# vita-epfl/motion-style-transfer

Measured on AMD Instinct MI355X. Metric: trajectories/sec fwd+bwd (Y-Net+LoRA, SDD shortterm), higher is better.
Workload: dtype f32; 1 GPU; C2: SDD shortterm Y-Net + LoRA rank=1 on encoder[0-4], 256x256 raster, obs=8 pred=12; batch_per_gpu=32, global_batch=32, raster=256x256, obs_len=8, pred_len=12, train_net=mosa_1, parallelism=dp1, trainable_floats=8190

## Files before the change

motion-style-transfer_amd/csrc/lora_wgrad.hip:

```cpp
#include "ynet_common.h"
#include <stdlib.h>
#include <stdio.h>
#include <type_traits>

#define LW_RQ 3
#define LW_ROWS 9

struct LoraWgArgs {
    YSrc src[YNET_MAX_SRC];
    int nsrc, cin;
    const float* dy;
    long long dy_bs;
    const float* mask;
    long long mask_bs;
    const float* lora_a;
    const float* lora_b;
    float* partial;
    int B, H, W, cout;
    int tiles_x, tiles_y, ntiles;
#ifdef YNET_LW_PROFILE
    unsigned long long* prof;
#endif
};

#ifdef YNET_LW_PROFILE
#define LW_STAMP(i) do { __builtin_amdgcn_sched_barrier(0); unsigned long long t_; asm volatile("s_waitcnt vmcnt(0) lgkmcnt(0)\n\ts_memtime %0\n\ts_waitcnt lgkmcnt(0)" : "=s"(t_) :: "memory"); pr[i] += t_ - tp; tp = t_; __builtin_amdgcn_sched_barrier(0); } while (0)
#else
#define LW_STAMP(i) do { } while (0)
#endif

typedef __attribute__((address_space(3))) void* lw_lds_ptr_t;
typedef const __attribute__((address_space(4))) float* lw_const_f32;

template <int TH>
struct LwCfg {
    static constexpr int TW = 32, NPIX = TH * TW, NH = 256 / NPIX;
    static constexpr int TROWS = TH + 2, TCOLS = 40;
    static constexpr int XDATA = TROWS * TCOLS / 4;
    static constexpr int XQ = (XDATA + 1 + 6) / 8 * 8 + 1;
    static constexpr int XCH = XQ * 4;
    static constexpr int DCH = NPIX + 4;
    static constexpr int PL = NPIX + 4;
    static_assert(XCH % 32 == 4 && DCH % 32 == 4, "bank-spread strides");
    static_assert(NH == 2 || NH == 4, "256 threads = NH slices of the tile's pixels");
    static constexpr int KSTEPS = NPIX / 4;
};

static inline int lw_xq(int th) { return ((th + 2) * 10 + 1 + 6) / 8 * 8 + 1; }
static inline int lw_lds_floats(int th, int cin, int cout) {
    const int npix = th * 32;
    return cin * lw_xq(th) * 4 + 64 + cout * (npix + 4) + 2 * LW_ROWS * (npix + 4) + cout * 12 + cin * 28;
}

__device__ __forceinline__ void lw_dma16(__amdgpu_buffer_rsrc_t r, const float* lds, unsigned voff) {
    __builtin_amdgcn_raw_ptr_buffer_load_lds(r, (lw_lds_ptr_t)lds, 16, voff, 0, 0, 0);
}

template <int TH, int NTG, int COS, int CIN_T, int COUT_T>
__global__ __launch_bounds__(256, (TH == 2 && COS <= 8) ? 3 : 2) void lora_wgrad_kernel(const LoraWgArgs a) {
    using C = LwCfg<TH>;
    constexpr int NPIX = C::NPIX, NH = C::NH, TCOLS = C::TCOLS, XQ = C::XQ, XCH = C::XCH, DCH = C::DCH, PL = C::PL;
    extern __shared__ __attribute__((aligned(16))) float smem[];
    const int cin = CIN_T ? CIN_T : a.cin, cout = COUT_T ? COUT_T : a.cout;
    float* xs = smem;
    float* ds = xs + cin * XCH + 64;
    float* dpl = ds + cout * DCH;
    float* xpl = dpl + LW_ROWS * PL;
    float* tb = xpl + LW_ROWS * PL;
    float* ta = tb + cout * 12;

    const int tid = threadIdx.x, lane = tid & 63;
    const int wave = __builtin_amdgcn_readfirstlane(tid >> 6);
    const int H = a.H, W = a.W, HW = H * W;
    const unsigned plane_bytes = (unsigned)HW * 4u;
    const int ncol = 9 * cin;
    const int n3 = 3 * cin;
    const lw_const_f32 la = (lw_const_f32)a.lora_a;

    const int NE = (cout + 15) >> 4;
    const int r16 = lane & 15, kq = lane >> 4;
    int gbase[NTG];
#pragma unroll
    for (int j = 0; j < NTG; ++j) {
        int u = (wave + 4 * j) * 16 + r16;
        u = u < ncol ? u : ncol - 1;
        const int ci = u / 9, t = u - 9 * ci, ky = t / 3, kx = t - 3 * ky;
        gbase[j] = ci * XCH + ky * TCOLS + kx + 3 + kq;
    }
    int eco = wave * 16 + r16;
    eco = eco < cout ? eco : cout - 1;
    const int ebase = eco * DCH + kq;
    const int arow = (r16 < LW_ROWS ? r16 : LW_ROWS - 1) * PL + kq;
    const bool has_e = wave < NE;

    f32x4 accg[NTG], acce = {0.f, 0.f, 0.f, 0.f};
#pragma unroll
    for (int j = 0; j < NTG; ++j) accg[j] = f32x4{0.f, 0.f, 0.f, 0.f};

    const int p = tid & (NPIX - 1);
    const int h = __builtin_amdgcn_readfirstlane(tid / NPIX);
    const int prow = p >> 5, pcol = p & 31;
    const int xoff_p = prow * TCOLS + pcol + 3;

    constexpr int XI_MAX = TH == 4 ? 9 : 11;
    const int nquads = cin * XQ;
    int xrc[XI_MAX];
    unsigned xcoff[XI_MAX];
    int xsid[XI_MAX];
#pragma unroll
    for (int k = 0; k < XI_MAX; ++k) {
        const int q = tid + k * 256;
        const int ch = q / XQ, within = q - ch * XQ;
        const int row = within / (TCOLS / 4), colp = (within - row * (TCOLS / 4)) * 4;
        int c = ch, sid = -1;
        if (q < nquads && within < C::XDATA) {
#pragma unroll
            for (int s_ = 0; s_ < YNET_MAX_SRC; ++s_) {
                if (sid < 0 && s_ < a.nsrc) {
                    if (c < a.src[s_].c) sid = s_;
                    else c -= a.src[s_].c;
                }
            }
        }
        xrc[k] = sid >= 0 ? (row << 8 | colp) : -1;
        xcoff[k] = (unsigned)c * plane_bytes;
        xsid[k] = sid;
    }

    for (int i = tid; i < cout * 12; i += 256) {
        const int co = i / 12, m = i - 12 * co;
        tb[i] = m < LW_ROWS ? a.lora_b[9 * co + m] : 0.f;
    }
    for (int i = tid; i < cin * 28; i += 256) {
        const int ci = i / 28, j = i - 28 * ci, q = j / 9, tp = j - 9 * q;
        const int ii = (9 * ci) / n3;
        const int n = 9 * ci + tp - ii * n3;
        ta[i] = (j < 27 && n < n3) ? a.lora_a[q * n3 + n] : 0.f;
    }

    float dyv[COS], mkv[COS];
    auto fetch_dy = [&](int tile) {
        int t = tile;
        const int x0 = (t % a.tiles_x) * 32;
        t /= a.tiles_x;
        const int y0 = (t % a.tiles_y) * TH;
        const int b = t / a.tiles_y;
        const int gy = y0 + prow, gx = x0 + pcol;
        const bool inside = gy < H && gx < W;
        const long long pix = (long long)gy * W + gx;
        const float* dyp = a.dy + (long long)b * a.dy_bs + pix;
        const float* mkp = a.mask ? a.mask + (long long)b * a.mask_bs + pix : nullptr;
#pragma unroll
        for (int k = 0; k < COS; ++k) {
            const int co = h + k * NH;
            const bool ok = inside && co < cout;
            dyv[k] = ok ? dyp[(long long)co * HW] : 0.f;
            mkv[k] = (ok && mkp) ? mkp[(long long)co * HW] : 1.f;
        }
    };
    if ((int)blockIdx.x < a.ntiles) fetch_dy(blockIdx.x);
#ifdef YNET_LW_PROFILE
    unsigned long long pr[8] = {0, 0, 0, 0, 0, 0, 0, 0}, tp = __builtin_amdgcn_s_memtime();
    const unsigned long long t_begin = tp;
#endif

    for (int tile = blockIdx.x; tile < a.ntiles; tile += gridDim.x) {
        int t = tile;
        const int x0 = (t % a.tiles_x) * 32;
        t /= a.tiles_x;
        const int y0 = (t % a.tiles_y) * TH;
        const int b = t / a.tiles_y;

        {
            unsigned xo[XI_MAX];
#pragma unroll
            for (int k = 0; k < XI_MAX; ++k) {
                const int gy = y0 + (xrc[k] >> 8) - 1, gx = x0 + (xrc[k] & 255) - 4;
                const bool ok = xrc[k] >= 0 && gy >= 0 && gy < H && gx >= 0 && gx < W;
                xo[k] = ok ? xcoff[k] + (unsigned)(gy * W + gx) * 4u : 0x80000000u;
            }
#pragma unroll 1
            for (int s_ = 0; s_ < a.nsrc; ++s_) {
                const float* base = a.src[s_].p + (long long)b * a.src[s_].bs;
                const unsigned long long ub = (unsigned long long)base;
                const unsigned lo = __builtin_amdgcn_readfirstlane((unsigned)ub), hi = __builtin_amdgcn_readfirstlane((unsigned)(ub >> 32));
                const __amdgpu_buffer_rsrc_t r = __builtin_amdgcn_make_buffer_rsrc(
                    (void*)(((unsigned long long)hi << 32) | lo), 0, (unsigned)a.src[s_].c * plane_bytes, 0x00020000);
#pragma unroll
                for (int k = 0; k < XI_MAX; ++k) {
                    if (k * 256 < nquads) {
                        const int with_src = xo[k] == 0x80000000u ? 0 : xsid[k];
                        if (tid + k * 256 < nquads && with_src == s_) lw_dma16(r, xs + (k * 256 + wave * 64) * 4, xo[k]);
                    }
                }
            }
        }
        LW_STAMP(0);
        float dp[LW_ROWS], xp[LW_ROWS];
#pragma unroll
        for (int m = 0; m < LW_ROWS; ++m) dp[m] = xp[m] = 0.f;
#pragma unroll
        for (int k = 0; k < COS; ++k) {
            const int co = h + k * NH;
            if (co < cout) {
                const float d = mkv[k] > 0.f ? dyv[k] : 0.f;
                ds[co * DCH + p] = d;
                const f32x4* cb = reinterpret_cast<const f32x4*>(tb + co * 12);
                const f32x4 c0 = cb[0], c1 = cb[1], c2 = cb[2];
#pragma unroll
                for (int m = 0; m < LW_ROWS; ++m)
                    dp[m] = __builtin_fmaf(m < 4 ? c0[m & 3] : (m < 8 ? c1[m & 3] : c2[m & 3]), d, dp[m]);
            }
        }
        LW_STAMP(1);
        asm volatile("s_waitcnt vmcnt(0)" ::: "memory");
        __syncthreads();
        LW_STAMP(2);

        {
            const float* xb = xs + xoff_p;
#pragma unroll
            for (int ii = 0; ii < 3; ++ii) {
                float s0 = 0.f, s1 = 0.f, s2 = 0.f;
                const int lo_u = ii * n3, hi_u = lo_u + n3;
                const int ci_lo = (lo_u + 8) / 9, ci_hi = hi_u / 9;
                const int head_end = min(9 * ci_lo, hi_u);
                const int tail_begin = max(9 * ci_hi, head_end);
#pragma unroll 2
                for (int ci = ci_lo + h; ci < ci_hi; ci += NH) {
                    const float* xc = xb + ci * XCH;
                    const f32x4* cv = reinterpret_cast<const f32x4*>(ta + ci * 28);
                    float cf[28], xv[9];
#pragma unroll
                    for (int j = 0; j < 7; ++j) {
                        const f32x4 c4 = cv[j];
                        cf[4 * j] = c4[0];
                        cf[4 * j + 1] = c4[1];
                        cf[4 * j + 2] = c4[2];
                        cf[4 * j + 3] = c4[3];
                    }
#pragma unroll
                    for (int t = 0; t < 9; ++t) xv[t] = xc[(t / 3) * TCOLS + (t % 3)];
#pragma unroll
                    for (int t = 0; t < 9; ++t) {
                        s0 = __builtin_fmaf(cf[t], xv[t], s0);
                        s1 = __builtin_fmaf(cf[9 + t], xv[t], s1);
                        s2 = __builtin_fmaf(cf[18 + t], xv[t], s2);
                    }
                }
                if (h == 0) {
                    auto one = [&](int u) {
                        const int ci = u / 9, tp = u - 9 * ci, ky = tp / 3, kx = tp - 3 * ky, n = u - lo_u;
                        const float xv = xb[ci * XCH + ky * TCOLS + kx];
                        s0 = __builtin_fmaf(la[n], xv, s0);
                        s1 = __builtin_fmaf(la[n3 + n], xv, s1);
                        s2 = __builtin_fmaf(la[2 * n3 + n], xv, s2);
                    };
#pragma unroll 1
                    for (int u = lo_u; u < head_end; ++u) one(u);
#pragma unroll 1
                    for (int u = tail_begin; u < hi_u; ++u) one(u);
                }
                xp[3 * ii + 0] = s0;
                xp[3 * ii + 1] = s1;
                xp[3 * ii + 2] = s2;
            }
        }
        LW_STAMP(3);
#pragma unroll
        for (int hh = 0; hh < NH; ++hh) {
            if (h == hh) {
#pragma unroll
                for (int m = 0; m < LW_ROWS; ++m) {
                    if (hh == 0) {
                        dpl[m * PL + p] = dp[m];
                        xpl[m * PL + p] = xp[m];
                    } else {
                        dpl[m * PL + p] += dp[m];
                        xpl[m * PL + p] += xp[m];
                    }
                }
            }
            __syncthreads();
        }

        LW_STAMP(4);
        if (tile + (int)gridDim.x < a.ntiles) fetch_dy(tile + gridDim.x);

        LW_STAMP(5);
        {
            const float* a_dp = dpl + arow;
            const float* a_xp = xpl + arow;
            const float* b_e = ds + ebase;
            const float* b_g[NTG];
#pragma unroll
            for (int j = 0; j < NTG; ++j) b_g[j] = xs + gbase[j];
            auto run = [&](auto with_e) {
                constexpr bool WE = decltype(with_e)::value;
                float ac, bc[NTG], ec = 0.f, dc = 0.f, an, bn[NTG], en = 0.f, dn = 0.f;
                ac = a_dp[0];
#pragma unroll
                for (int j = 0; j < NTG; ++j) bc[j] = b_g[j][0];
                if (WE) {
                    ec = a_xp[0];
                    dc = b_e[0];
                }
#pragma unroll
                for (int s_ = 0; s_ < C::KSTEPS; ++s_) {
                    if (s_ + 1 < C::KSTEPS) {
                        const int sn = s_ + 1, xo = (sn >> 3) * TCOLS + (sn & 7) * 4;
                        an = a_dp[4 * sn];
#pragma unroll
                        for (int j = 0; j < NTG; ++j) bn[j] = b_g[j][xo];
                        if (WE) {
                            en = a_xp[4 * sn];
                            dn = b_e[4 * sn];
                        }
                    }
                    __builtin_amdgcn_sched_barrier(0);
#pragma unroll
                    for (int j = 0; j < NTG; ++j) accg[j] = __builtin_amdgcn_mfma_f32_16x16x4f32(ac, bc[j], accg[j], 0, 0, 0);
                    if (WE) acce = __builtin_amdgcn_mfma_f32_16x16x4f32(ec, dc, acce, 0, 0, 0);
                    __builtin_amdgcn_sched_barrier(0);
                    ac = an;
#pragma unroll
                    for (int j = 0; j < NTG; ++j) bc[j] = bn[j];
                    if (WE) {
                        ec = en;
                        dc = dn;
                    }
                }
            };
            if (has_e) run(std::true_type{});
            else run(std::false_type{});
        }
        LW_STAMP(6);
        __syncthreads();
        LW_STAMP(7);
    }
#ifdef YNET_LW_PROFILE
    if (lane == 0) {
        for (int i = 0; i < 8; ++i) atomicAdd(a.prof + i, pr[i]);
        atomicAdd(a.prof + 8, __builtin_amdgcn_s_memtime() - t_begin);
        atomicAdd(a.prof + 9, 1ull);
    }
#endif

    float* pg = a.partial + (long long)blockIdx.x * (LW_ROWS * (ncol + cout));
    float* pe = pg + LW_ROWS * ncol;
#pragma unroll
    for (int j = 0; j < NTG; ++j) {
        const int u = (wave + 4 * j) * 16 + r16;
        if (u < ncol) {
#pragma unroll
            for (int e = 0; e < 4; ++e) {
                const int m = 4 * kq + e;
                if (m < LW_ROWS) pg[m * ncol + u] = accg[j][e];
            }
        }
    }
    if (has_e) {
        const int co = wave * 16 + r16;
        if (co < cout) {
#pragma unroll
            for (int e = 0; e < 4; ++e) {
                const int m = 4 * kq + e;
                if (m < LW_ROWS) pe[m * cout + co] = acce[e];
            }
        }
    }
}

__global__ __launch_bounds__(256) void lora_wgrad_reduce_kernel(const float* __restrict__ partial, int nwg, int cin, int cout,
                                                                float scale, float* __restrict__ d_a, float* __restrict__ d_b) {
    __shared__ float red[8][32];
    const int o = threadIdx.x & 31, g = threadIdx.x >> 5;
    const int n3 = 3 * cin, ncol = 9 * cin, na = LW_RQ * n3, nb = 9 * cout;
    const long long stride = (long long)LW_ROWS * (ncol + cout);
    for (int base = blockIdx.x * 32; base < na + nb; base += gridDim.x * 32) {
        const int i = base + o;
        float s0 = 0.f, s1 = 0.f, s2 = 0.f;
        if (i < na) {
            const int q = i / n3, n = i - q * n3;
            const float* p0 = partial + (0 * LW_RQ + q) * ncol + 0 * n3 + n;
            const float* p1 = partial + (1 * LW_RQ + q) * ncol + 1 * n3 + n;
            const float* p2 = partial + (2 * LW_RQ + q) * ncol + 2 * n3 + n;
            int w = g;
            for (; w + 24 < nwg; w += 32) {
                float t0 = 0.f, t1 = 0.f, t2 = 0.f;
#pragma unroll
                for (int k = 0; k < 4; ++k) {
                    t0 += p0[(w + 8 * k) * stride];
                    t1 += p1[(w + 8 * k) * stride];
                    t2 += p2[(w + 8 * k) * stride];
                }
                s0 += t0;
                s1 += t1;
                s2 += t2;
            }
            for (; w < nwg; w += 8) {
                s0 += p0[w * stride];
                s1 += p1[w * stride];
                s2 += p2[w * stride];
            }
        } else if (i < na + nb) {
            const int f = i - na, co = f / 9, m = f - 9 * co;
            const float* p0 = partial + (long long)LW_ROWS * ncol + m * cout + co;
            int w = g;
            for (; w + 56 < nwg; w += 64) {
                float t0 = 0.f, t1 = 0.f;
#pragma unroll
                for (int k = 0; k < 4; ++k) {
                    t0 += p0[(w + 8 * k) * stride];
                    t1 += p0[(w + 32 + 8 * k) * stride];
                }
                s0 += t0;
                s1 += t1;
            }
            for (; w < nwg; w += 8) s0 += p0[w * stride];
        }
        red[g][o] = (s0 + s1) + s2;
        __syncthreads();
        if (g == 0 && i < na + nb) {
            float t = red[0][o];
#pragma unroll
            for (int k = 1; k < 8; ++k) t += red[k][o];
            if (i < na) d_a[i] = scale * t;
            else d_b[i - na] = scale * t;
        }
        __syncthreads();
    }
}

static int lw_tile_rows(int cin, int cout) {
    if (cin <= 32 && cout <= 32) return 4;
    if (cin <= 64 && cout <= 64) return 2;
    return 0;
}

static int lw_grid(int ntiles, int lds_bytes) {
    int dev = 0, cus = 256;
    (void)hipGetDevice(&dev);
    (void)hipDeviceGetAttribute(&cus, hipDeviceAttributeMultiprocessorCount, dev);
    if (cus < 1) cus = 256;
    int per_cu = (160 * 1024) / lds_bytes;
    static const int cap = getenv("YNET_LW_WG_PER_CU") ? atoi(getenv("YNET_LW_WG_PER_CU")) : 3;
    if (per_cu > cap) per_cu = cap;
    if (per_cu < 1) per_cu = 1;
    const int slots = per_cu * cus;
    return ntiles < slots ? ntiles : slots;
}

template <int TH, int NTG, int COS, int CIN_T = 0, int COUT_T = 0>
static int launch_lora_wgrad(const LoraWgArgs& a, int grid, hipStream_t st) {
    static bool attr_dev[YNET_MAX_DEV] = {false};
    bool& attr_set = attr_dev[ynet_device_slot()];
    if (!attr_set) {
        (void)hipFuncSetAttribute(reinterpret_cast<const void*>(lora_wgrad_kernel<TH, NTG, COS, CIN_T, COUT_T>), hipFuncAttributeMaxDynamicSharedMemorySize, 160 * 1024);
        attr_set = true;
    }
    const int lds = lw_lds_floats(TH, a.cin, a.cout) * 4;
#ifdef YNET_LW_PROFILE
    static unsigned long long* prof_dev = nullptr;
    if (!prof_dev) (void)hipMalloc(&prof_dev, 128);
    (void)hipMemsetAsync(prof_dev, 0, 128, st);
    LoraWgArgs ap = a;
    ap.prof = prof_dev;
    hipLaunchKernelGGL((lora_wgrad_kernel<TH, NTG, COS, CIN_T, COUT_T>), dim3(grid), dim3(256), lds, st, ap);
    {
        unsigned long long h[16];
        (void)hipMemcpyAsync(h, prof_dev, 128, hipMemcpyDeviceToHost, st);
        (void)hipStreamSynchronize(st);
        const double tot = (double)h[8];
        static const char* nm[8] = {"dma-issue", "DP", "dma-wait+barrier", "XP", "combine", "dy-prefetch", "MFMA", "end-barrier"};
        fprintf(stderr, "lora_wgrad<%d,%d,%d,%d,%d> grid %d tiles %d waves %llu avg cycles/wave %.0f:", TH, NTG, COS, CIN_T, COUT_T, grid, a.ntiles, h[9], tot / (double)h[9]);
        for (int i = 0; i < 8; ++i) fprintf(stderr, " %s %.1f%%", nm[i], 100.0 * (double)h[i] / tot);
        fprintf(stderr, "\n");
    }
#else
    hipLaunchKernelGGL((lora_wgrad_kernel<TH, NTG, COS, CIN_T, COUT_T>), dim3(grid), dim3(256), lds, st, a);
#endif
    return ynet_check_launch("lora_conv2d_wgrad");
}

extern "C" {

int ynet_lora_conv2d_wgrad_supported(int cin, int cout, int K, int r, int W) {
    static const int on = getenv("YNET_LORA_WGRAD") ? atoi(getenv("YNET_LORA_WGRAD")) : 1;
    return (on && K == 3 && r == 1 && cin >= 1 && cout >= 1 && (W & 3) == 0 && lw_tile_rows(cin, cout) != 0) ? 1 : 0;
}

int ynet_lora_conv2d_wgrad_preferred(int cin, int cout, int K, int r, int W) {
    static const int on = getenv("YNET_LORA_WGRAD") ? atoi(getenv("YNET_LORA_WGRAD")) : 1;
    if (!ynet_lora_conv2d_wgrad_supported(cin, cout, K, r, W)) return 0;
    return (on >= 2 || cout > 32) ? 1 : 0;
}

long long ynet_lora_conv2d_wgrad_workspace_floats(int cin, int cout) {
    return 1024ll * LW_ROWS * (9ll * cin + cout);
}

int ynet_lora_conv2d_wgrad(const float* const* src, const int* src_c, const long long* src_bs, int nsrc,
                           const float* dy, long long dy_bs, const float* mask, long long mask_bs,
                           const float* lora_a, const float* lora_b, float scale, float* d_a, float* d_b,
                           float* workspace, int B, int H, int W, int cout, int K, int r, void* stream) {
    YNET_REQUIRE(nsrc >= 1 && nsrc <= YNET_MAX_SRC, "lora_conv2d_wgrad: 1..%d sources supported", YNET_MAX_SRC);
    YNET_REQUIRE(dy && lora_a && lora_b && d_a && d_b && workspace, "lora_conv2d_wgrad: null pointer");
    YNET_REQUIRE(B > 0 && H > 0 && W > 0 && cout > 0, "lora_conv2d_wgrad: empty problem");
    LoraWgArgs a{};
    a.nsrc = nsrc;
    a.cin = 0;
    auto misaligned = [](const void* p, long long bs) { return (reinterpret_cast<uintptr_t>(p) & 15) != 0 || (bs & 3) != 0; };
    for (int i = 0; i < nsrc; ++i) {
        YNET_REQUIRE(src[i] != nullptr && src_c[i] > 0, "lora_conv2d_wgrad: source %d is null/empty", i);
        YNET_REQUIRE(!misaligned(src[i], src_bs[i]), "lora_conv2d_wgrad: source %d is not 16-byte aligned", i);
        a.src[i] = YSrc{src[i], src_c[i], src_bs[i], 0};
        a.cin += src_c[i];
    }
    YNET_REQUIRE(ynet_lora_conv2d_wgrad_supported(a.cin, cout, K, r, W), "lora_conv2d_wgrad: cin %d cout %d K %d r %d W %d is not served (3x3, r = 1, channels <= 64, W %% 4 == 0)", a.cin, cout, K, r, W);
    static const int th2_all = getenv("YNET_LW_TH2") ? atoi(getenv("YNET_LW_TH2")) : 0;
    const int th = th2_all ? 2 : lw_tile_rows(a.cin, cout);
    a.dy = dy;
    a.dy_bs = dy_bs;
    a.mask = mask;
    a.mask_bs = mask_bs;
    a.lora_a = lora_a;
    a.lora_b = lora_b;
    a.partial = workspace;
    a.B = B;
    a.H = H;
    a.W = W;
    a.cout = cout;
    a.tiles_x = ceil_div(W, 32);
    a.tiles_y = ceil_div(H, th);
    a.ntiles = B * a.tiles_x * a.tiles_y;
    YNET_REQUIRE(a.cin * lw_xq(th) <= (th == 4 ? 9 : 11) * 256, "lora_conv2d_wgrad: x tile of %d channels exceeds the DMA plan", a.cin);
    const int grid = lw_grid(a.ntiles, lw_lds_floats(th, a.cin, cout) * 4);
    hipStream_t st = (hipStream_t)stream;
    const int ntg = ceil_div(ceil_div(9 * a.cin, 16), 4);
    int rc;
    if (th == 2 && a.cin == 14 && cout == 32) rc = launch_lora_wgrad<2, 2, 8, 14, 32>(a, grid, st);
    else if (th == 2 && a.cin == 32 && cout == 32) rc = launch_lora_wgrad<2, 5, 8, 32, 32>(a, grid, st);
    else if (th == 2 && a.cin == 32 && cout == 64) rc = launch_lora_wgrad<2, 5, 16, 32, 64>(a, grid, st);
    else if (a.cin == 14 && cout == 32) rc = launch_lora_wgrad<4, 2, 16, 14, 32>(a, grid, st);
    else if (a.cin == 32 && cout == 32) rc = launch_lora_wgrad<4, 5, 16, 32, 32>(a, grid, st);
    else if (a.cin == 32 && cout == 64) rc = launch_lora_wgrad<4, 5, 32, 32, 64>(a, grid, st);
    else if (a.cin == 64 && cout == 64) rc = launch_lora_wgrad<2, 9, 16, 64, 64>(a, grid, st);
    else if (th == 4) {
        if (cout <= 32) rc = ntg <= 2 ? launch_lora_wgrad<4, 2, 16>(a, grid, st) : launch_lora_wgrad<4, 5, 16>(a, grid, st);
        else rc = ntg <= 2 ? launch_lora_wgrad<4, 2, 32>(a, grid, st) : launch_lora_wgrad<4, 5, 32>(a, grid, st);
    } else {
        rc = launch_lora_wgrad<2, 9, 16>(a, grid, st);
    }
    if (rc) return rc;
    const int nout = LW_RQ * 3 * a.cin + 9 * cout;
    hipLaunchKernelGGL(lora_wgrad_reduce_kernel, dim3(ceil_div(nout, 32)), dim3(256), 0, st, workspace, grid, a.cin, cout, scale, d_a, d_b);
    return ynet_check_launch("lora_conv2d_wgrad(reduce)");
}

}
```

Before: 4979 trajectories/s.

## Rework LoRA weight-grad kernel: compact partials, wider reduce, earlier dy prefetch

The LoRA weight-gradient kernel now reads lora_a coefficients straight from constant memory instead of staging them in LDS, and keeps only a small LDS table for the boundary terms. It moves the next tile's dy prefetch ahead of the per-slice pixel reduction, and replaces the serialized slice-by-slice LDS accumulation with copy buffers whenever they fit without lowering occupancy. Per-workgroup partials keep only the 3 relevant rows for the A gradient, and the reduce kernel uses 1024 threads with one block per output group. Together these aim to cut LDS traffic, barriers, workspace size and reduce-pass latency, at the cost of more LDS and more complex code.

```diff
diff --git a/motion-style-transfer_amd/csrc/lora_wgrad.hip b/motion-style-transfer_amd/csrc/lora_wgrad.hip
--- a/motion-style-transfer_amd/csrc/lora_wgrad.hip
+++ b/motion-style-transfer_amd/csrc/lora_wgrad.hip
@@ -5,6 +5,7 @@
 
 #define LW_RQ 3
 #define LW_ROWS 9
+#define LW_MAX_WG 1024
 
 struct LoraWgArgs {
     YSrc src[YNET_MAX_SRC];
@@ -18,6 +19,7 @@
     float* partial;
     int B, H, W, cout;
     int tiles_x, tiles_y, ntiles;
+    int copies;
 #ifdef YNET_LW_PROFILE
     unsigned long long* prof;
 #endif
@@ -49,8 +51,10 @@
 static inline int lw_xq(int th) { return ((th + 2) * 10 + 1 + 6) / 8 * 8 + 1; }
 static inline int lw_lds_floats(int th, int cin, int cout) {
     const int npix = th * 32;
-    return cin * lw_xq(th) * 4 + 64 + cout * (npix + 4) + 2 * LW_ROWS * (npix + 4) + cout * 12 + cin * 28;
-}
+    return cin * lw_xq(th) * 4 + 64 + cout * (npix + 4) + 2 * LW_ROWS * (npix + 4) + cout * 12 + 192;
+}
+static inline int lw_copy_floats(int th) { return (256 / (th * 32) - 2) * 2 * LW_ROWS * th * 32; }
+
 
 __device__ __forceinline__ void lw_dma16(__amdgpu_buffer_rsrc_t r, const float* lds, unsigned voff) {
     __builtin_amdgcn_raw_ptr_buffer_load_lds(r, (lw_lds_ptr_t)lds, 16, voff, 0, 0, 0);
@@ -67,7 +71,8 @@
     float* dpl = ds + cout * DCH;
     float* xpl = dpl + LW_ROWS * PL;
     float* tb = xpl + LW_ROWS * PL;
-    float* ta = tb + cout * 12;
+    float* ts = tb + cout * 12;
+    float* cp = ts + 192;
 
     const int tid = threadIdx.x, lane = tid & 63;
     const int wave = __builtin_amdgcn_readfirstlane(tid >> 6);
@@ -127,15 +132,25 @@
         xsid[k] = sid;
     }
 
-    for (int i = tid; i < cout * 12; i += 256) {
-        const int co = i / 12, m = i - 12 * co;
-        tb[i] = m < LW_ROWS ? a.lora_b[9 * co + m] : 0.f;
-    }
-    for (int i = tid; i < cin * 28; i += 256) {
-        const int ci = i / 28, j = i - 28 * ci, q = j / 9, tp = j - 9 * q;
-        const int ii = (9 * ci) / n3;
-        const int n = 9 * ci + tp - ii * n3;
-        ta[i] = (j < 27 && n < n3) ? a.lora_a[q * n3 + n] : 0.f;
+    constexpr int TB_IT = 64 * 12 / 256;
+    float tbv[TB_IT];
+#pragma unroll
+    for (int k = 0; k < TB_IT; ++k) {
+        const int i = tid + 256 * k, co = i / 12, m = i - 12 * co;
+        const bool ok = i < cout * 12 && m < LW_ROWS;
+        const float v = a.lora_b[ok ? 9 * co + m : 0];
+        tbv[k] = ok ? v : 0.f;
+    }
+    float tsv;
+    {
+        const int ii = tid >> 6, j = (tid >> 2) & 15, q = tid & 3;
+        const int lo_u = ii * n3, hi_u = lo_u + n3;
+        const int head_end = min(9 * ((lo_u + 8) / 9), hi_u), tail_begin = max(9 * (hi_u / 9), head_end);
+        const int nh = head_end - lo_u;
+        const int u = j < nh ? lo_u + j : tail_begin + (j - nh);
+        const bool ok = tid < 192 && q < 3 && u < hi_u;
+        const float v = a.lora_a[ok ? q * n3 + (u - lo_u) : 0];
+        tsv = ok ? v : 0.f;
     }
 
     float dyv[COS], mkv[COS];
@@ -159,6 +174,11 @@
         }
     };
     if ((int)blockIdx.x < a.ntiles) fetch_dy(blockIdx.x);
+#pragma unroll
+    for (int k = 0; k < TB_IT; ++k)
+        if (tid + 256 * k < cout * 12) tb[tid + 256 * k] = tbv[k];
+    if (tid < 192) ts[tid] = tsv;
+    __syncthreads();
 #ifdef YNET_LW_PROFILE
     unsigned long long pr[8] = {0, 0, 0, 0, 0, 0, 0, 0}, tp = __builtin_amdgcn_s_memtime();
     const unsigned long long t_begin = tp;
@@ -170,6 +190,13 @@
         t /= a.tiles_x;
         const int y0 = (t % a.tiles_y) * TH;
         const int b = t / a.tiles_y;
+
+        float dv[COS];
+#pragma unroll
+        for (int k = 0; k < COS; ++k) {
+            dv[k] = mkv[k] > 0.f ? dyv[k] : 0.f;
+            asm volatile("" : "+v"(dv[k])::"memory");
+        }
 
         {
             unsigned xo[XI_MAX];
@@ -203,7 +230,7 @@
         for (int k = 0; k < COS; ++k) {
             const int co = h + k * NH;
             if (co < cout) {
-                const float d = mkv[k] > 0.f ? dyv[k] : 0.f;
+                const float d = dv[k];
                 ds[co * DCH + p] = d;
                 const f32x4* cb = reinterpret_cast<const f32x4*>(tb + co * 12);
                 const f32x4 c0 = cb[0], c1 = cb[1], c2 = cb[2];
@@ -216,6 +243,8 @@
         asm volatile("s_waitcnt vmcnt(0)" ::: "memory");
         __syncthreads();
         LW_STAMP(2);
+        if (tile + (int)gridDim.x < a.ntiles) fetch_dy(tile + gridDim.x);
+        LW_STAMP(5);
 
         {
             const float* xb = xs + xoff_p;
@@ -229,37 +258,39 @@
 #pragma unroll 2
                 for (int ci = ci_lo + h; ci < ci_hi; ci += NH) {
                     const float* xc = xb + ci * XCH;
-                    const f32x4* cv = reinterpret_cast<const f32x4*>(ta + ci * 28);
-                    float cf[28], xv[9];
-#pragma unroll
-                    for (int j = 0; j < 7; ++j) {
-                        const f32x4 c4 = cv[j];
-                        cf[4 * j] = c4[0];
-                        cf[4 * j + 1] = c4[1];
-                        cf[4 * j + 2] = c4[2];
-                        cf[4 * j + 3] = c4[3];
+                    const lw_const_f32 c0 = la + (9 * ci - lo_u), c1 = c0 + n3, c2 = c1 + n3;
+                    float xv[9];
+#pragma unroll
+                    for (int t = 0; t < 9; ++t) xv[t] = xc[(t / 3) * TCOLS + (t % 3)];
+#pragma unroll
+                    for (int t = 0; t < 9; ++t) {
+                        s0 = __builtin_fmaf(c0[t], xv[t], s0);
+                        s1 = __builtin_fmaf(c1[t], xv[t], s1);
+                        s2 = __builtin_fmaf(c2[t], xv[t], s2);
                     }
-#pragma unroll
-                    for (int t = 0; t < 9; ++t) xv[t] = xc[(t / 3) * TCOLS + (t % 3)];
-#pragma unroll
-                    for (int t = 0; t < 9; ++t) {
-                        s0 = __builtin_fmaf(cf[t], xv[t], s0);
-                        s1 = __builtin_fmaf(cf[9 + t], xv[t], s1);
-                        s2 = __builtin_fmaf(cf[18 + t], xv[t], s2);
+                }
+                if (h == 0) {
+                    const f32x4* cs = reinterpret_cast<const f32x4*>(ts) + ii * 16;
+                    const int nh = head_end - lo_u;
+                    auto one = [&](int u, int j) {
+                        const int ci = u / 9, tp = u - 9 * ci, ky = tp / 3, kx = tp - 3 * ky;
+                        const float xv = xb[ci * XCH + ky * TCOLS + kx];
+                        const f32x4 c4 = cs[j];
+                        s0 = __builtin_fmaf(c4[0], xv, s0);
+                        s1 = __builtin_fmaf(c4[1], xv, s1);
+                        s2 = __builtin_fmaf(c4[2], xv, s2);
+                    };
+                    if constexpr (CIN_T != 0) {
+#pragma unroll
+                        for (int u = lo_u; u < head_end; ++u) one(u, u - lo_u);
+#pragma unroll
+                        for (int u = tail_begin; u < hi_u; ++u) one(u, nh + u - tail_begin);
+                    } else {
+#pragma unroll 1
+                        for (int u = lo_u; u < head_end; ++u) one(u, u - lo_u);
+#pragma unroll 1
+                        for (int u = tail_begin; u < hi_u; ++u) one(u, nh + u - tail_begin);
                     }
-                }
-                if (h == 0) {
-                    auto one = [&](int u) {
-                        const int ci = u / 9, tp = u - 9 * ci, ky = tp / 3, kx = tp - 3 * ky, n = u - lo_u;
-                        const float xv = xb[ci * XCH + ky * TCOLS + kx];
-                        s0 = __builtin_fmaf(la[n], xv, s0);
-                        s1 = __builtin_fmaf(la[n3 + n], xv, s1);
-                        s2 = __builtin_fmaf(la[2 * n3 + n], xv, s2);
-                    };
-#pragma unroll 1
-                    for (int u = lo_u; u < head_end; ++u) one(u);
-#pragma unroll 1
-                    for (int u = tail_begin; u < hi_u; ++u) one(u);
                 }
                 xp[3 * ii + 0] = s0;
                 xp[3 * ii + 1] = s1;
@@ -267,27 +298,57 @@
             }
         }
         LW_STAMP(3);
-#pragma unroll
-        for (int hh = 0; hh < NH; ++hh) {
-            if (h == hh) {
+        if (NH > 2 && a.copies) {
+            if (h == 1) {
 #pragma unroll
                 for (int m = 0; m < LW_ROWS; ++m) {
-                    if (hh == 0) {
-                        dpl[m * PL + p] = dp[m];
-                        xpl[m * PL + p] = xp[m];
-                    } else {
-                        dpl[m * PL + p] += dp[m];
-                        xpl[m * PL + p] += xp[m];
+                    dpl[m * PL + p] = dp[m];
+                    xpl[m * PL + p] = xp[m];
+                }
+            } else if (h >= 2) {
+                float* c = cp + (h - 2) * (2 * LW_ROWS * NPIX) + p;
+#pragma unroll
+                for (int m = 0; m < LW_ROWS; ++m) {
+                    c[m * NPIX] = dp[m];
+                    c[(LW_ROWS + m) * NPIX] = xp[m];
+                }
+            }
+            __syncthreads();
+            if (h == 0) {
+#pragma unroll
+                for (int m = 0; m < LW_ROWS; ++m) {
+                    float d = dp[m] + dpl[m * PL + p], x = xp[m] + xpl[m * PL + p];
+#pragma unroll
+                    for (int hh = 2; hh < NH; ++hh) {
+                        const float* c = cp + (hh - 2) * (2 * LW_ROWS * NPIX) + p;
+                        d += c[m * NPIX];
+                        x += c[(LW_ROWS + m) * NPIX];
                     }
+                    dpl[m * PL + p] = d;
+                    xpl[m * PL + p] = x;
                 }
             }
             __syncthreads();
+        } else {
+#pragma unroll
+            for (int hh = 0; hh < NH; ++hh) {
+                if (h == hh) {
+#pragma unroll
+                    for (int m = 0; m < LW_ROWS; ++m) {
+                        if (hh == 0) {
+                            dpl[m * PL + p] = dp[m];
+                            xpl[m * PL + p] = xp[m];
+                        } else {
+                            dpl[m * PL + p] += dp[m];
+                            xpl[m * PL + p] += xp[m];
+                        }
+                    }
+                }
+                __syncthreads();
+            }
         }
 
         LW_STAMP(4);
-        if (tile + (int)gridDim.x < a.ntiles) fetch_dy(tile + gridDim.x);
-
-        LW_STAMP(5);
         {
             const float* a_dp = dpl + arow;
             const float* a_xp = xpl + arow;
@@ -346,16 +407,17 @@
     }
 #endif
 
-    float* pg = a.partial + (long long)blockIdx.x * (LW_ROWS * (ncol + cout));
-    float* pe = pg + LW_ROWS * ncol;
+    float* pg = a.partial + (long long)blockIdx.x * (LW_RQ * ncol + LW_ROWS * cout);
+    float* pe = pg + LW_RQ * ncol;
 #pragma unroll
     for (int j = 0; j < NTG; ++j) {
         const int u = (wave + 4 * j) * 16 + r16;
         if (u < ncol) {
+            const int m0 = (u / n3) * LW_RQ;
 #pragma unroll
             for (int e = 0; e < 4; ++e) {
                 const int m = 4 * kq + e;
-                if (m < LW_ROWS) pg[m * ncol + u] = accg[j][e];
+                if (m >= m0 && m < m0 + LW_RQ) pg[(m - m0) * ncol + u] = accg[j][e];
             }
         }
     }
@@ -365,70 +427,68 @@
 #pragma unroll
             for (int e = 0; e < 4; ++e) {
                 const int m = 4 * kq + e;
-                if (m < LW_ROWS) pe[m * cout + co] = acce[e];
-            }
-        }
-    }
-}
-
-__global__ __launch_bounds__(256) void lora_wgrad_reduce_kernel(const float* __restrict__ partial, int nwg, int cin, int cout,
-                                                                float scale, float* __restrict__ d_a, float* __restrict__ d_b) {
-    __shared__ float red[8][32];
-    const int o = threadIdx.x & 31, g = threadIdx.x >> 5;
-    const int n3 = 3 * cin, ncol = 9 * cin, na = LW_RQ * n3, nb = 9 * cout;
-    const long long stride = (long long)LW_ROWS * (ncol + cout);
-    for (int base = blockIdx.x * 32; base < na + nb; base += gridDim.x * 32) {
-        const int i = base + o;
-        float s0 = 0.f, s1 = 0.f, s2 = 0.f;
-        if (i < na) {
-            const int q = i / n3, n = i - q * n3;
-            const float* p0 = partial + (0 * LW_RQ + q) * ncol + 0 * n3 + n;
-            const float* p1 = partial + (1 * LW_RQ + q) * ncol + 1 * n3 + n;
-            const float* p2 = partial + (2 * LW_RQ + q) * ncol + 2 * n3 + n;
-            int w = g;
-            for (; w + 24 < nwg; w += 32) {
-                float t0 = 0.f, t1 = 0.f, t2 = 0.f;
-#pragma unroll
-                for (int k = 0; k < 4; ++k) {
-                    t0 += p0[(w + 8 * k) * stride];
-                    t1 += p1[(w + 8 * k) * stride];
-                    t2 += p2[(w + 8 * k) * stride];
-                }
-                s0 += t0;
-                s1 += t1;
-                s2 += t2;
-            }
-            for (; w < nwg; w += 8) {
-                s0 += p0[w * stride];
-                s1 += p1[w * stride];
-                s2 += p2[w * stride];
-            }
-        } else if (i < na + nb) {
-            const int f = i - na, co = f / 9, m = f - 9 * co;
-            const float* p0 = partial + (long long)LW_ROWS * ncol + m * cout + co;
-            int w = g;
-            for (; w + 56 < nwg; w += 64) {
-                float t0 = 0.f, t1 = 0.f;
-#pragma unroll
-                for (int k = 0; k < 4; ++k) {
-                    t0 += p0[(w + 8 * k) * stride];
-                    t1 += p0[(w + 32 + 8 * k) * stride];
-                }
-                s0 += t0;
-                s1 += t1;
-            }
-            for (; w < nwg; w += 8) s0 += p0[w * stride];
-        }
-        red[g][o] = (s0 + s1) + s2;
-        __syncthreads();
-        if (g == 0 && i < na + nb) {
-            float t = red[0][o];
-#pragma unroll
-            for (int k = 1; k < 8; ++k) t += red[k][o];
-            if (i < na) d_a[i] = scale * t;
-            else d_b[i - na] = scale * t;
-        }
-        __syncthreads();
+                if (m < LW_ROWS) pe[co * LW_ROWS + m] = acce[e];
+            }
+        }
+    }
+}
+
+#define LW_RED_O 32
+#define LW_RED_G 32
+__global__ __launch_bounds__(LW_RED_O * LW_RED_G) void lora_wgrad_reduce_kernel(const float* __restrict__ partial, int nwg, int cin, int cout,
+                                                                                 float scale, float* __restrict__ d_a, float* __restrict__ d_b) {
+    __shared__ float red[LW_RED_G][LW_RED_O + 1];
+    const int o = threadIdx.x & (LW_RED_O - 1), g = threadIdx.x / LW_RED_O;
+    const int n3 = 3 * cin, ncol = 9 * cin, na = LW_RQ * n3, nb = LW_ROWS * cout;
+    const long long stride = (long long)LW_RQ * ncol + nb;
+    const int i = blockIdx.x * LW_RED_O + o;
+    float s0 = 0.f, s1 = 0.f, s2 = 0.f;
+    if (i < na) {
+        const int q = i / n3, n = i - q * n3;
+        const float* p0 = partial + q * ncol + n;
+        int w = g;
+        for (; w + 7 * LW_RED_G < nwg; w += 8 * LW_RED_G) {
+            float t0 = 0.f, t1 = 0.f, t2 = 0.f;
+#pragma unroll
+            for (int k = 0; k < 8; ++k) {
+                const float* pw = p0 + (w + LW_RED_G * k) * stride;
+                t0 += pw[0];
+                t1 += pw[n3];
+                t2 += pw[2 * n3];
+            }
+            s0 += t0;
+            s1 += t1;
+            s2 += t2;
+        }
+        for (; w < nwg; w += LW_RED_G) {
+            const float* pw = p0 + w * stride;
+            s0 += pw[0];
+            s1 += pw[n3];
+            s2 += pw[2 * n3];
+        }
+    } else if (i < na + nb) {
+        const float* p0 = partial + (long long)LW_RQ * ncol + (i - na);
+        int w = g;
+        for (; w + 7 * LW_RED_G < nwg; w += 8 * LW_RED_G) {
+            float t0 = 0.f, t1 = 0.f;
+#pragma unroll
+            for (int k = 0; k < 4; ++k) {
+                t0 += p0[(w + LW_RED_G * k) * stride];
+                t1 += p0[(w + LW_RED_G * (4 + k)) * stride];
+            }
+            s0 += t0;
+            s1 += t1;
+        }
+        for (; w < nwg; w += LW_RED_G) s0 += p0[w * stride];
+    }
+    red[g][o] = (s0 + s1) + s2;
+    __syncthreads();
+    if (g == 0 && i < na + nb) {
+        float t = red[0][o];
+#pragma unroll
+        for (int k = 1; k < LW_RED_G; ++k) t += red[k][o];
+        if (i < na) d_a[i] = scale * t;
+        else d_b[i - na] = scale * t;
     }
 }
 
@@ -438,28 +498,37 @@
     return 0;
 }
 
-static int lw_grid(int ntiles, int lds_bytes) {
-    int dev = 0, cus = 256;
-    (void)hipGetDevice(&dev);
-    (void)hipDeviceGetAttribute(&cus, hipDeviceAttributeMultiprocessorCount, dev);
-    if (cus < 1) cus = 256;
+static int lw_per_cu(int lds_bytes) {
     int per_cu = (160 * 1024) / lds_bytes;
     static const int cap = getenv("YNET_LW_WG_PER_CU") ? atoi(getenv("YNET_LW_WG_PER_CU")) : 3;
     if (per_cu > cap) per_cu = cap;
-    if (per_cu < 1) per_cu = 1;
-    const int slots = per_cu * cus;
+    return per_cu < 1 ? 1 : per_cu;
+}
+
+static int lw_lds_bytes(int th, int cin, int cout, int* copies) {
+    const int base = lw_lds_floats(th, cin, cout) * 4, with = base + lw_copy_floats(th) * 4;
+    *copies = (lw_copy_floats(th) > 0 && lw_per_cu(with) == lw_per_cu(base)) ? 1 : 0;
+    return *copies ? with : base;
+}
+
+static int lw_grid(int ntiles, int lds_bytes) {
+    static int cus_dev[YNET_MAX_DEV] = {0};
+    const int slot = ynet_device_slot();
+    int& cus = cus_dev[slot];
+    if (cus < 1 && (hipDeviceGetAttribute(&cus, hipDeviceAttributeMultiprocessorCount, slot) != hipSuccess || cus < 1)) cus = 256;
+    const int per_cu = lw_per_cu(lds_bytes);
+    const int slots = per_cu * cus < LW_MAX_WG ? per_cu * cus : LW_MAX_WG;
     return ntiles < slots ? ntiles : slots;
 }
 
 template <int TH, int NTG, int COS, int CIN_T = 0, int COUT_T = 0>
-static int launch_lora_wgrad(const LoraWgArgs& a, int grid, hipStream_t st) {
+static int launch_lora_wgrad(const LoraWgArgs& a, int grid, int lds, hipStream_t st) {
     static bool attr_dev[YNET_MAX_DEV] = {false};
     bool& attr_set = attr_dev[ynet_device_slot()];
     if (!attr_set) {
         (void)hipFuncSetAttribute(reinterpret_cast<const void*>(lora_wgrad_kernel<TH, NTG, COS, CIN_T, COUT_T>), hipFuncAttributeMaxDynamicSharedMemorySize, 160 * 1024);
         attr_set = true;
     }
-    const int lds = lw_lds_floats(TH, a.cin, a.cout) * 4;
 #ifdef YNET_LW_PROFILE
     static unsigned long long* prof_dev = nullptr;
     if (!prof_dev) (void)hipMalloc(&prof_dev, 128);
@@ -497,7 +566,7 @@
 }
 
 long long ynet_lora_conv2d_wgrad_workspace_floats(int cin, int cout) {
-    return 1024ll * LW_ROWS * (9ll * cin + cout);
+    return (long long)LW_MAX_WG * (LW_RQ * 9ll * cin + LW_ROWS * (long long)cout);
 }
 
 int ynet_lora_conv2d_wgrad(const float* const* src, const int* src_c, const long long* src_bs, int nsrc,
@@ -535,26 +604,27 @@
     a.tiles_y = ceil_div(H, th);
     a.ntiles = B * a.tiles_x * a.tiles_y;
     YNET_REQUIRE(a.cin * lw_xq(th) <= (th == 4 ? 9 : 11) * 256, "lora_conv2d_wgrad: x tile of %d channels exceeds the DMA plan", a.cin);
-    const int grid = lw_grid(a.ntiles, lw_lds_floats(th, a.cin, cout) * 4);
+    const int lds = lw_lds_bytes(th, a.cin, cout, &a.copies);
+    const int grid = lw_grid(a.ntiles, lds);
     hipStream_t st = (hipStream_t)stream;
     const int ntg = ceil_div(ceil_div(9 * a.cin, 16), 4);
     int rc;
-    if (th == 2 && a.cin == 14 && cout == 32) rc = launch_lora_wgrad<2, 2, 8, 14, 32>(a, grid, st);
-    else if (th == 2 && a.cin == 32 && cout == 32) rc = launch_lora_wgrad<2, 5, 8, 32, 32>(a, grid, st);
-    else if (th == 2 && a.cin == 32 && cout == 64) rc = launch_lora_wgrad<2, 5, 16, 32, 64>(a, grid, st);
-    else if (a.cin == 14 && cout == 32) rc = launch_lora_wgrad<4, 2, 16, 14, 32>(a, grid, st);
-    else if (a.cin == 32 && cout == 32) rc = launch_lora_wgrad<4, 5, 16, 32, 32>(a, grid, st);
-    else if (a.cin == 32 && cout == 64) rc = launch_lora_wgrad<4, 5, 32, 32, 64>(a, grid, st);
-    else if (a.cin == 64 && cout == 64) rc = launch_lora_wgrad<2, 9, 16, 64, 64>(a, grid, st);
+    if (th == 2 && a.cin == 14 && cout == 32) rc = launch_lora_wgrad<2, 2, 8, 14, 32>(a, grid, lds, st);
+    else if (th == 2 && a.cin == 32 && cout == 32) rc = launch_lora_wgrad<2, 5, 8, 32, 32>(a, grid, lds, st);
+    else if (th == 2 && a.cin == 32 && cout == 64) rc = launch_lora_wgrad<2, 5, 16, 32, 64>(a, grid, lds, st);
+    else if (a.cin == 14 && cout == 32) rc = launch_lora_wgrad<4, 2, 16, 14, 32>(a, grid, lds, st);
+    else if (a.cin == 32 && cout == 32) rc = launch_lora_wgrad<4, 5, 16, 32, 32>(a, grid, lds, st);
+    else if (a.cin == 32 && cout == 64) rc = launch_lora_wgrad<4, 5, 32, 32, 64>(a, grid, lds, st);
+    else if (a.cin == 64 && cout == 64) rc = launch_lora_wgrad<2, 9, 16, 64, 64>(a, grid, lds, st);
     else if (th == 4) {
-        if (cout <= 32) rc = ntg <= 2 ? launch_lora_wgrad<4, 2, 16>(a, grid, st) : launch_lora_wgrad<4, 5, 16>(a, grid, st);
-        else rc = ntg <= 2 ? launch_lora_wgrad<4, 2, 32>(a, grid, st) : launch_lora_wgrad<4, 5, 32>(a, grid, st);
+        if (cout <= 32) rc = ntg <= 2 ? launch_lora_wgrad<4, 2, 16>(a, grid, lds, st) : launch_lora_wgrad<4, 5, 16>(a, grid, lds, st);
+        else rc = ntg <= 2 ? launch_lora_wgrad<4, 2, 32>(a, grid, lds, st) : launch_lora_wgrad<4, 5, 32>(a, grid, lds, st);
     } else {
-        rc = launch_lora_wgrad<2, 9, 16>(a, grid, st);
+        rc = launch_lora_wgrad<2, 9, 16>(a, grid, lds, st);
     }
     if (rc) return rc;
     const int nout = LW_RQ * 3 * a.cin + 9 * cout;
-    hipLaunchKernelGGL(lora_wgrad_reduce_kernel, dim3(ceil_div(nout, 32)), dim3(256), 0, st, workspace, grid, a.cin, cout, scale, d_a, d_b);
+    hipLaunchKernelGGL(lora_wgrad_reduce_kernel, dim3(ceil_div(nout, LW_RED_O)), dim3(LW_RED_O * LW_RED_G), 0, st, workspace, grid, a.cin, cout, scale, d_a, d_b);
     return ynet_check_launch("lora_conv2d_wgrad(reduce)");
 }
 
```

Measured after the change: 4977 trajectories/s. About the same (-0.0%).
